# HITSZ-NRSL/De6D

Hardware: AMD Instinct MI355X
Metric: scenes/sec (16384-pt KITTI) at 1/2/4/8 MI355X; 3D mAP parity vs ref (higher is better)
Workload: dtype f32

## Files before the change

de6d_amd/csrc/mlp_chain.hip:

```cpp
#include "common.h"
#include <stdlib.h>

namespace {

D6_GEMM_PRIO_DECL

typedef float f32x16 __attribute__((ext_vector_type(16)));

constexpr int kChainWaves = 4;
constexpr int kPackTiles = 1;
constexpr int kTS = 33;
constexpr int kMaxK1 = 8;
constexpr int kMaxC = 32;
constexpr int kMaxC3 = 64;

struct ChainArgs {
  int rows;
  int n, m, ns;
  const float *a; int lda;
  const int *idx;
  const float *ctr; int ldctr;
  const int *cnt;
  const float *w1, *w2, *w3;
  int ldw1, ldw2, ldw3;
  const float *s1, *s2, *s3;
  int k1, c1, c2, c3;
  float *y; int ldy; int col0;
  const int *hdr; const int *crow_p; const int *crow_c;
};

__device__ __forceinline__ int compact_class(int row0, int h1, int h2, int h3, int h4, int h5) {
  return row0 < h1 ? 32 : row0 < h2 ? 16 : row0 < h3 ? 8 : row0 < h4 ? 4 : row0 < h5 ? 2 : 1;
}
__device__ __forceinline__ int compact_out_row(int s, int qq, int kh) {
  if (s < 4) return -1;
  if (s == 4) return 8 * qq + 4 * kh;
  if (kh) return -1;
  if (s == 8) return 8 * qq;
  if (s == 16) return (qq & 1) ? -1 : 8 * qq;
  return qq == 0 ? 0 : -1;
}
__device__ __forceinline__ void compact_store(float *dst, float val, int tag) {
  if (tag & 0x20000000) __hip_atomic_fetch_max(reinterpret_cast<int *>(dst), __builtin_bit_cast(int, val), __ATOMIC_RELAXED, __HIP_MEMORY_SCOPE_AGENT);
  else *dst = val;
}
__device__ __forceinline__ void compact_store_small(const ChainArgs &g, const f32x16 &o, int s, const int (&tags)[16], int col, float sh) {
#pragma unroll
  for (int e = 0; e < 16; ++e) {
    if (s == 2 && (e & 1)) continue;
    const float raw = s == 2 ? d6_vmax(o[e], o[e + 1 < 16 ? e + 1 : e]) : o[e];
    const int tag = tags[e];
    if (tag >= 0) compact_store(g.y + (size_t)(tag & 0x1fffffff) * g.ldy + g.col0 + col, (tag & 0x40000000) ? 0.f : d6_relu(raw + sh), tag);
  }
}
__device__ __forceinline__ void compact_row_tags(int my_tag, int kh, int (&tags)[16]) {
#pragma unroll
  for (int e = 0; e < 16; ++e) tags[e] = __shfl(my_tag, (e & 3) + 8 * (e >> 2) + 4 * kh);
}
__device__ __forceinline__ void compact_pool(float (&v)[4], int s) {
  if (s == 4) return;
#pragma unroll
  for (int qq = 0; qq < 4; ++qq) v[qq] = d6_vmax(v[qq], __shfl_xor(v[qq], 32));
  if (s == 16) {
    v[0] = d6_vmax(v[0], v[1]);
    v[2] = d6_vmax(v[2], v[3]);
  } else if (s == 32) {
    v[0] = d6_vmax(d6_vmax(v[0], v[1]), d6_vmax(v[2], v[3]));
  }
}

__device__ __forceinline__ float relu1(float v) { return v > 0.f ? v : 0.f; }

__host__ __device__ __forceinline__ int chain_col(int j, int k1) { return j + 3 < k1 ? j + 3 : j + 3 - k1; }

__global__ __launch_bounds__(64 * kChainWaves) void mlp_chain_kernel(const ChainArgs g) {
  D6_GEMM_PRIO_APPLY();
  __shared__ float W1[kMaxK1 * kMaxC];
  __shared__ float W2[kMaxC * kMaxC];
  __shared__ float W3[kMaxC * kMaxC3];
  __shared__ float S1[kMaxC], S2[kMaxC], S3[kMaxC3];
  __shared__ float T[kChainWaves][2][kMaxC * kTS];

  const int tid = threadIdx.x, lane = tid & 63, wave = tid >> 6;
  const int l31 = lane & 31, kh = lane >> 5;

  for (int t = tid; t < kMaxK1 * kMaxC; t += blockDim.x) {
    const int k = t / kMaxC, c = t % kMaxC;
    W1[t] = (k < g.k1 && c < g.c1) ? g.w1[(size_t)chain_col(k, g.k1) * g.ldw1 + c] : 0.f;
  }
  for (int t = tid; t < kMaxC * kMaxC; t += blockDim.x) {
    const int k = t / kMaxC, c = t % kMaxC;
// ... 94 lines not shown
      if (j >= nt3) break;
      const int col = 32 * j + l31;
      const bool cok = col < g.c3;
      const float sh = S3[col];
      float q[4];
#pragma unroll
      for (int qq = 0; qq < 4; ++qq) {
        float mx = relu1(acc3[j][4 * qq] + sh);
#pragma unroll
        for (int e = 1; e < 4; ++e) {
          const float v = relu1(acc3[j][4 * qq + e] + sh);
          mx = v > mx ? v : mx;
        }
        const float o = __shfl_xor(mx, 32);
        q[qq] = o > mx ? o : mx;
      }
      if (g.ns == 32) {
        float mx = q[0];
        mx = q[1] > mx ? q[1] : mx; mx = q[2] > mx ? q[2] : mx; mx = q[3] > mx ? q[3] : mx;
        if (cok && kh == 0) g.y[(size_t)tile * g.ldy + g.col0 + col] = (g.cnt[tile] > 0) ? mx : 0.f;
      } else {
        const float m0 = q[1] > q[0] ? q[1] : q[0];
        const float m1 = q[3] > q[2] ? q[3] : q[2];
        if (cok && kh == 0) {
          g.y[(size_t)(2 * tile) * g.ldy + g.col0 + col] = (g.cnt[2 * tile] > 0) ? m0 : 0.f;
          g.y[(size_t)(2 * tile + 1) * g.ldy + g.col0 + col] = (g.cnt[2 * tile + 1] > 0) ? m1 : 0.f;
        }
      }
    }
    __builtin_amdgcn_wave_barrier();
  }
}

template <int C1, int C2, int C3, int NS, bool COMPACT = false>
__global__ __launch_bounds__(256) void mlp_chain_reg_kernel(const ChainArgs g) {
  D6_GEMM_PRIO_APPLY();
  constexpr int S1 = 2;
  constexpr int S2 = C1 / 2, S3 = C2 / 2, NT3 = C3 / 32;
  const int lane = threadIdx.x & 63, l31 = lane & 31, kh = lane >> 5;
  int wave_global = (blockIdx.x * blockDim.x + threadIdx.x) >> 6;
  int n_waves = (gridDim.x * blockDim.x) >> 6;
  int pk_end = 0;
  if (COMPACT) {
    const int wpw = blockDim.x >> 6, live = g.hdr[0] / 32;
    int nb = (live + wpw * kPackTiles - 1) / (wpw * kPackTiles);
    if (nb > (int)gridDim.x) nb = gridDim.x;
    if ((int)blockIdx.x >= nb) return;
    n_waves = nb * wpw;
    pk_end = live;
  }

  float wf1[S1 + 1], wf2[S2 + 1], wf3[NT3][S3];
#pragma unroll
  for (int s = 0; s < S1; ++s) wf1[s] = l31 < C1 ? g.w1[(size_t)chain_col(2 * s + kh, 4) * g.ldw1 + l31] : 0.f;
  wf1[S1] = (kh == 0 && l31 < C1) ? g.s1[l31] : 0.f;
#pragma unroll
  for (int s = 0; s < S2; ++s) wf2[s] = l31 < C2 ? g.w2[(size_t)(2 * s + kh) * g.ldw2 + l31] : 0.f;
  wf2[S2] = (kh == 0 && l31 < C2) ? g.s2[l31] : 0.f;
#pragma unroll
  for (int j = 0; j < NT3; ++j)
#pragma unroll
    for (int s = 0; s < S3; ++s) wf3[j][s] = g.w3[(size_t)(2 * s + kh) * g.ldw3 + 32 * j + l31];
  float sh3[NT3];
#pragma unroll
  for (int j = 0; j < NT3; ++j) sh3[j] = g.s3[32 * j + l31];
  const float one_k0 = kh == 0 ? 1.f : 0.f;

  int h1 = 0, h2 = 0, h3 = 0, h4 = 0, h5 = 0;
  if (COMPACT) { h1 = g.hdr[1]; h2 = g.hdr[2]; h3 = g.hdr[3]; h4 = g.hdr[4]; h5 = g.hdr[5]; }
  const int ntiles = COMPACT ? pk_end : g.rows / 32;
  const int *nb_idx = COMPACT ? g.crow_p : g.idx;
  int tile = __builtin_amdgcn_readfirstlane(wave_global);
  if (tile >= ntiles) return;
  struct TileIn { float4 row; float cx, cy, cz; int cnt0, cnt1; int oc[4]; int tag; };
  struct TileIdx { int p, cj; };
  auto fetch_idx = [&](int t) {
    TileIdx ix;
    ix.p = nb_idx[t * 32 + l31];
    ix.cj = COMPACT ? g.crow_c[t * 32 + l31] : 0;
    return ix;
  };
  auto fetch = [&](int t, const TileIdx &ix) {
    TileIn in;
    const int p = ix.p;
    if (COMPACT) {
      in.row = *reinterpret_cast<const float4 *>(g.a + (size_t)p * 4);
      const int cj = ix.cj;
      const float *c = g.ctr + (size_t)(cj < 0 ? 0 : cj & 0x1fffffff) * g.ldctr;
      in.cx = c[0]; in.cy = c[1]; in.cz = c[2];
      in.cnt0 = in.cnt1 = 0;
      in.tag = cj;
      const int sc = compact_class(t * 32, h1, h2, h3, h4, h5);
#pragma unroll
      for (int qq = 0; qq < 4; ++qq) {
        const int r = compact_out_row(sc, qq, kh);
        const int tg = __shfl(cj, r < 0 ? 0 : r);
        in.oc[qq] = r >= 0 ? tg : -1;
      }
      return in;
    }
    in.tag = 0;
    const int c0 = NS == 32 ? t : 2 * t;
    const int bi = c0 / g.m;
    const int cj = NS == 32 ? c0 : c0 + (l31 >> 4);
    in.row = *reinterpret_cast<const float4 *>(g.a + ((size_t)bi * g.n + p) * 4);
    const float *c = g.ctr + (size_t)cj * g.ldctr;
    in.cx = c[0]; in.cy = c[1]; in.cz = c[2];
    in.cnt0 = g.cnt[c0];
    in.cnt1 = NS == 32 ? 0 : g.cnt[c0 + 1];
    return in;
  };
  TileIn nxt = fetch(tile, fetch_idx(tile));
  TileIdx ix_next = tile + n_waves < ntiles ? fetch_idx(tile + n_waves) : TileIdx{0, 0};
  float pend[NT3][COMPACT ? 4 : 2];
  int pend_oc[4] = {-1, -1, -1, -1};
  int pend_tile = -1;
  auto flush = [&]() {
#pragma unroll
    for (int j = 0; j < NT3; ++j) {
      const int col = 32 * j + l31;
      if (COMPACT) {
#pragma unroll
        for (int qq = 0; qq < 4; ++qq)
          if (pend_oc[qq] >= 0) compact_store(g.y + (size_t)(pend_oc[qq] & 0x1fffffff) * g.ldy + g.col0 + col, pend[j][qq], pend_oc[qq]);
      } else if (NS == 32) {
        g.y[(size_t)pend_tile * g.ldy + g.col0 + col] = pend[j][0];
      } else {
        g.y[(size_t)(2 * pend_tile) * g.ldy + g.col0 + col] = pend[j][0];
        g.y[(size_t)(2 * pend_tile + 1) * g.ldy + g.col0 + col] = pend[j][1];
      }
    }
  };
  for (; tile < ntiles; tile += n_waves) {
    const TileIn cur = nxt;
    if (pend_tile >= 0) flush();
    if (tile + n_waves < ntiles) {
      nxt = fetch(tile + n_waves, ix_next);
      if (tile + 2 * n_waves < ntiles) ix_next = fetch_idx(tile + 2 * n_waves);
    }
    const float4 v0 = cur.row;
    const float cx = cur.cx, cy = cur.cy, cz = cur.cz;
    const float x0 = v0.x - cx, x1 = v0.y - cy, x2 = v0.z - cz, x3 = v0.w;

    f32x16 acc;
#pragma unroll
    for (int e = 0; e < 16; ++e) acc[e] = 0.f;
    acc = __builtin_amdgcn_mfma_f32_32x32x2f32(wf1[0], kh ? x0 : x3, acc, 0, 0, 0);
    acc = __builtin_amdgcn_mfma_f32_32x32x2f32(wf1[1], kh ? x2 : x1, acc, 0, 0, 0);
    acc = __builtin_amdgcn_mfma_f32_32x32x2f32(wf1[2], one_k0, acc, 0, 0, 0);
    float frag[16];
    auto to_fragments = [&](const f32x16 &a, int nreg) {
#pragma unroll
      for (int G = 0; G < 4; ++G) {
        if (4 * G >= nreg) break;
        float t[4];
#pragma unroll
        for (int e = 0; e < 4; ++e) t[e] = d6_relu(a[4 * G + e]);
        asm volatile("s_nop 1\n\tv_permlane32_swap_b32 %0, %1\n\ts_nop 1\n\tv_permlane32_swap_b32 %2, %3\n\ts_nop 1"
                     : "+v"(t[0]), "+v"(t[1]), "+v"(t[2]), "+v"(t[3]));
        frag[4 * G + 0] = t[0];
        frag[4 * G + 1] = t[2];
        frag[4 * G + 2] = t[1];
        frag[4 * G + 3] = t[3];
      }
    };
    to_fragments(acc, S2);
#pragma unroll
    for (int e = 0; e < 16; ++e) acc[e] = 0.f;
#pragma unroll
    for (int s = 0; s < S2; ++s) acc = __builtin_amdgcn_mfma_f32_32x32x2f32(wf2[s], frag[s], acc, 0, 0, 0);
    acc = __builtin_amdgcn_mfma_f32_32x32x2f32(wf2[S2], one_k0, acc, 0, 0, 0);
    to_fragments(acc, S3);
#pragma unroll
    for (int j = 0; j < NT3; ++j) {
      f32x16 o;
#pragma unroll
      for (int e = 0; e < 16; ++e) o[e] = 0.f;
#pragma unroll
      for (int s = 0; s < S3; ++s) o = __builtin_amdgcn_mfma_f32_32x32x2f32(frag[s], wf3[j][s], o, 0, 0, 0);
      const int col = 32 * j + l31;
      float q[4];
      if (COMPACT) {
#pragma unroll
        for (int qq = 0; qq < 4; ++qq) q[qq] = d6_vmax(d6_vmax(o[4 * qq], o[4 * qq + 1]), d6_vmax(o[4 * qq + 2], o[4 * qq + 3]));
        const int sc = compact_class(tile * 32, h1, h2, h3, h4, h5);
        if (sc < 4) {
          int tags[16];
          compact_row_tags(cur.tag, kh, tags);
          compact_store_small(g, o, sc, tags, col, sh3[j]);
#pragma unroll
          for (int qq = 0; qq < 4; ++qq) pend[j][qq] = 0.f;
          continue;
        }
        compact_pool(q, sc);
#pragma unroll
        for (int qq = 0; qq < 4; ++qq) pend[j][qq] = (cur.oc[qq] & 0x40000000) ? 0.f : d6_relu(q[qq] + sh3[j]);
        continue;
      }
#pragma unroll
      for (int qq = 0; qq < 4; ++qq) {
        const float mq = d6_vmax(d6_vmax(o[4 * qq], o[4 * qq + 1]), d6_vmax(o[4 * qq + 2], o[4 * qq + 3]));
        q[qq] = d6_vmax(mq, __shfl_xor(mq, 32));
      }
      if (NS == 32) {
        const float mx = d6_relu(d6_vmax(d6_vmax(q[0], q[1]), d6_vmax(q[2], q[3])) + sh3[j]);
        pend[j][0] = (cur.cnt0 > 0) ? mx : 0.f;
      } else {
        const float m0 = d6_relu(d6_vmax(q[0], q[1]) + sh3[j]);
        const float m1 = d6_relu(d6_vmax(q[2], q[3]) + sh3[j]);
        pend[j][0] = (cur.cnt0 > 0) ? m0 : 0.f;
        pend[j][1] = (cur.cnt1 > 0) ? m1 : 0.f;
      }
    }
    pend_tile = tile;
    if (COMPACT) {
#pragma unroll
      for (int qq = 0; qq < 4; ++qq) pend_oc[qq] = cur.oc[qq];
    }
  }
  flush();
}

template <int N, int STRIDE, bool W_IS_A>
__device__ __forceinline__ void mfma_steps_lds(const float *__restrict__ w, const float *x, f32x16 &acc) {
  constexpr int UB = 8, NB = (N + UB - 1) / UB;
  float wb[2][UB];
#pragma unroll
  for (int u = 0; u < UB; ++u)
    if (u < N) wb[0][u] = w[u * STRIDE];
#pragma unroll
  for (int b = 0; b < NB; ++b) {
    if (b + 1 < NB) {
#pragma unroll
      for (int u = 0; u < UB; ++u)
        if ((b + 1) * UB + u < N) wb[(b + 1) & 1][u] = w[((b + 1) * UB + u) * STRIDE];
    }
    __builtin_amdgcn_sched_barrier(0);
#pragma unroll
    for (int u = 0; u < UB; ++u) {
      if (b * UB + u < N) {
        if (W_IS_A) acc = __builtin_amdgcn_mfma_f32_32x32x2f32(wb[b & 1][u], x[b * UB + u], acc, 0, 0, 0);
        else acc = __builtin_amdgcn_mfma_f32_32x32x2f32(x[b * UB + u], wb[b & 1][u], acc, 0, 0, 0);
      }
    }
    __builtin_amdgcn_sched_barrier(0);
  }
}

template <int C2, int NS, bool COMPACT = false>
__global__ __launch_bounds__(512) void mlp_chain_wide_kernel(const ChainArgs g) {
  D6_GEMM_PRIO_APPLY();
  constexpr int K1 = 68, C1 = 64, C3 = 128;
  constexpr int S1 = K1 / 2, S2 = C1 / 2, S3 = C2 / 2;
  constexpr int T1 = C1 / 32, T2 = C2 / 32, T3 = C3 / 32;
  extern __shared__ float lds[];
  float *W1 = lds;
  float *W2 = W1 + (K1 + 2) * C1;
  float *W3 = W2 + (C1 + 2) * C2;
  const int tid = threadIdx.x, lane = tid & 63, l31 = lane & 31, kh = lane >> 5;
  int pk_stride = 0, pk_first = 0, pk_end = 0;
  if (COMPACT) {
    const int wpw = blockDim.x >> 6, live = g.hdr[0] / 32;
    int nb = (live + wpw * kPackTiles - 1) / (wpw * kPackTiles);
    if (nb > (int)gridDim.x) nb = gridDim.x;
    if ((int)blockIdx.x >= nb) return;
    pk_stride = nb * wpw;
    pk_first = blockIdx.x * wpw + (tid >> 6);
    pk_end = live;
  }
  auto stage = [&](float *dst, const float *w, int ldw, const float *shift, int k_rows, int cols, bool chain_order) {
    const int c4 = cols / 4;
    for (int t = tid; t < (k_rows + (shift ? 2 : 0)) * c4; t += blockDim.x) {
      const int k = t / c4, c = 4 * (t % c4);
      float4 v = make_float4(0.f, 0.f, 0.f, 0.f);
      if (k < k_rows) v = *reinterpret_cast<const float4 *>(w + (size_t)(chain_order ? chain_col(k, k_rows) : k) * ldw + c);
      else if (k == k_rows) v = *reinterpret_cast<const float4 *>(shift + c);
      *reinterpret_cast<float4 *>(dst + k * cols + c) = v;
    }
  };
  stage(W1, g.w1, g.ldw1, g.s1, K1, C1, true);
  stage(W2, g.w2, g.ldw2, g.s2, C1, C2, false);
  stage(W3, g.w3, g.ldw3, nullptr, C2, C3, false);
  float sh3[T3];
#pragma unroll
  for (int j = 0; j < T3; ++j) sh3[j] = g.s3[32 * j + l31];
  __syncthreads();

  const float one_k0 = kh == 0 ? 1.f : 0.f;
  const int wave_global = COMPACT ? pk_first : (int)((blockIdx.x * blockDim.x + tid) >> 6);
  const int n_waves = COMPACT ? pk_stride : (int)((gridDim.x * blockDim.x) >> 6);
  int h1 = 0, h2 = 0, h3 = 0, h4 = 0, h5 = 0;
  if (COMPACT) { h1 = g.hdr[1]; h2 = g.hdr[2]; h3 = g.hdr[3]; h4 = g.hdr[4]; h5 = g.hdr[5]; }
  const int ntiles = COMPACT ? pk_end : g.rows / 32;
  int tile = __builtin_amdgcn_readfirstlane(wave_global);
  if (tile >= ntiles) return;

  float xin[S1 + 1];
  float csub0, csub1;
  int cnt0, cnt1;
  int oc_n[4] = {-1, -1, -1, -1};
  int e_p = 0, e_c = 0, tag_n = 0;
  auto fetch_entries = [&](int t) {
    if (COMPACT) {
      e_p = g.crow_p[t * 32 + l31];
      e_c = g.crow_c[t * 32 + l31];
    } else {
      e_p = g.idx[t * 32 + l31];
    }
  };
  auto fetch = [&](int t) {
    if (COMPACT) {
      const int p = e_p;
      const float *row = g.a + (size_t)p * K1;
      const float *src = row + 3 + kh;
#pragma unroll
      for (int s = 0; s < S1 - 2; ++s) xin[s] = src[2 * s];
      xin[S1 - 2] = row[kh ? 0 : K1 - 1];
      xin[S1 - 1] = row[kh ? 2 : 1];
      const int cj = e_c;
      const float *c = g.ctr + (size_t)(cj < 0 ? 0 : cj & 0x1fffffff) * g.ldctr;
      csub0 = kh ? c[0] : 0.f;
      csub1 = kh ? c[2] : c[1];
      cnt0 = cnt1 = 0;
      tag_n = cj;
      const int sc = compact_class(t * 32, h1, h2, h3, h4, h5);
#pragma unroll
      for (int qq = 0; qq < 4; ++qq) {
        const int r = compact_out_row(sc, qq, kh);
        const int tg = __shfl(cj, r < 0 ? 0 : r);
        oc_n[qq] = r >= 0 ? tg : -1;
      }
      return;
    }
    const int c0 = NS == 32 ? t : 2 * t;
    const int bi = c0 / g.m;
    const int cj = NS == 32 ? c0 : c0 + (l31 >> 4);
    const int p = e_p;
    const float *row = g.a + ((size_t)bi * g.n + p) * K1;
    const float *src = row + 3 + kh;
#pragma unroll
    for (int s = 0; s < S1 - 2; ++s) xin[s] = src[2 * s];
    xin[S1 - 2] = row[kh ? 0 : K1 - 1];
    xin[S1 - 1] = row[kh ? 2 : 1];
    const float *c = g.ctr + (size_t)cj * g.ldctr;
    csub0 = kh ? c[0] : 0.f;
    csub1 = kh ? c[2] : c[1];
    cnt0 = g.cnt[c0];
    cnt1 = NS == 32 ? 0 : g.cnt[c0 + 1];
  };
  auto to_fragments = [&](const f32x16 &a, float *frag) {
#pragma unroll
    for (int G = 0; G < 4; ++G) {
      float t[4];
#pragma unroll
      for (int e = 0; e < 4; ++e) t[e] = d6_relu(a[4 * G + e]);
      asm volatile("s_nop 1\n\tv_permlane32_swap_b32 %0, %1\n\ts_nop 1\n\tv_permlane32_swap_b32 %2, %3\n\ts_nop 1"
                   : "+v"(t[0]), "+v"(t[1]), "+v"(t[2]), "+v"(t[3]));
      frag[4 * G + 0] = t[0]; frag[4 * G + 1] = t[2]; frag[4 * G + 2] = t[1]; frag[4 * G + 3] = t[3];
    }
  };

  float pend[T3][COMPACT ? 4 : 2];
  int pend_oc[4] = {-1, -1, -1, -1};
  int pend_tile = -1;
  auto flush = [&]() {
#pragma unroll
    for (int j = 0; j < T3; ++j) {
      const int col = 32 * j + l31;
      if (COMPACT) {
#pragma unroll
        for (int qq = 0; qq < 4; ++qq)
          if (pend_oc[qq] >= 0) compact_store(g.y + (size_t)(pend_oc[qq] & 0x1fffffff) * g.ldy + g.col0 + col, pend[j][qq], pend_oc[qq]);
      } else if (NS == 32) {
        g.y[(size_t)pend_tile * g.ldy + g.col0 + col] = pend[j][0];
      } else {
        g.y[(size_t)(2 * pend_tile) * g.ldy + g.col0 + col] = pend[j][0];
        g.y[(size_t)(2 * pend_tile + 1) * g.ldy + g.col0 + col] = pend[j][1];
      }
    }
  };

  fetch_entries(tile);
  fetch(tile);
  if (tile + n_waves < ntiles) fetch_entries(tile + n_waves);
  for (; tile < ntiles; tile += n_waves) {
    if (pend_tile >= 0) flush();
    const int my_cnt0 = cnt0, my_cnt1 = cnt1, my_tag = tag_n;
    int my_oc[4];
#pragma unroll
    for (int qq = 0; qq < 4; ++qq) my_oc[qq] = oc_n[qq];
    xin[S1 - 2] = xin[S1 - 2] - csub0;
    xin[S1 - 1] = xin[S1 - 1] - csub1;
    xin[S1] = one_k0;
    float f1[S2 + 1];
#pragma unroll
    for (int t = 0; t < T1; ++t) {
      f32x16 acc;
#pragma unroll
      for (int e = 0; e < 16; ++e) acc[e] = 0.f;
      mfma_steps_lds<S1 + 1, 2 * C1, true>(W1 + kh * C1 + 32 * t + l31, xin, acc);
      to_fragments(acc, f1 + 16 * t);
    }
    f1[S2] = one_k0;
    if (tile + n_waves < ntiles) {
      fetch(tile + n_waves);
      if (tile + 2 * n_waves < ntiles) fetch_entries(tile + 2 * n_waves);
    }
    float f2[S3];
#pragma unroll
    for (int t = 0; t < T2; ++t) {
      f32x16 acc;
#pragma unroll
      for (int e = 0; e < 16; ++e) acc[e] = 0.f;
      mfma_steps_lds<S2 + 1, 2 * C2, true>(W2 + kh * C2 + 32 * t + l31, f1, acc);
      to_fragments(acc, f2 + 16 * t);
    }
#pragma unroll
    for (int j = 0; j < T3; ++j) {
      f32x16 o;
#pragma unroll
      for (int e = 0; e < 16; ++e) o[e] = 0.f;
      mfma_steps_lds<S3, 2 * C3, false>(W3 + kh * C3 + 32 * j + l31, f2, o);
      float q[4];
      if (COMPACT) {
#pragma unroll
        for (int qq = 0; qq < 4; ++qq) q[qq] = d6_vmax(d6_vmax(o[4 * qq], o[4 * qq + 1]), d6_vmax(o[4 * qq + 2], o[4 * qq + 3]));
        const int sc = compact_class(tile * 32, h1, h2, h3, h4, h5);
        if (sc < 4) {
          int tags[16];
          compact_row_tags(my_tag, kh, tags);
          compact_store_small(g, o, sc, tags, 32 * j + l31, sh3[j]);
#pragma unroll
          for (int qq = 0; qq < 4; ++qq) pend[j][qq] = 0.f;
          continue;
        }
        compact_pool(q, sc);
#pragma unroll
        for (int qq = 0; qq < 4; ++qq) pend[j][qq] = (my_oc[qq] & 0x40000000) ? 0.f : d6_relu(q[qq] + sh3[j]);
        continue;
      }
#pragma unroll
      for (int qq = 0; qq < 4; ++qq) {
        const float mq = d6_vmax(d6_vmax(o[4 * qq], o[4 * qq + 1]), d6_vmax(o[4 * qq + 2], o[4 * qq + 3]));
        q[qq] = d6_vmax(mq, __shfl_xor(mq, 32));
      }
      if (NS == 32) {
        const float mx = d6_relu(d6_vmax(d6_vmax(q[0], q[1]), d6_vmax(q[2], q[3])) + sh3[j]);
        pend[j][0] = my_cnt0 > 0 ? mx : 0.f;
      } else {
        pend[j][0] = my_cnt0 > 0 ? d6_relu(d6_vmax(q[0], q[1]) + sh3[j]) : 0.f;
        pend[j][1] = my_cnt1 > 0 ? d6_relu(d6_vmax(q[2], q[3]) + sh3[j]) : 0.f;
      }
    }
    pend_tile = tile;
    if (COMPACT) {
#pragma unroll
      for (int qq = 0; qq < 4; ++qq) pend_oc[qq] = my_oc[qq];
    }
  }
  flush();
}

}

DET6D_API int det6d_mlp_chain3(int rows, int n, int m, int ns, const float *a, int lda, const int *idx,
                               const float *ctr, int ldctr, const int *cnt, const float *w1, int ldw1,
                               const float *s1, int c1, const float *w2, int ldw2, const float *s2, int c2,
                               const float *w3, int ldw3, const float *s3, int c3, float *y, int ldy, int col0,
                               det6d_stream_t stream) {
  D6_GEMM_PRIO_HOST();
  if (rows < 0 || n <= 0 || m <= 0 || (ns != 16 && ns != 32) || !a || !idx || !ctr || !cnt || !w1 || !w2 || !w3 ||
      !s1 || !s2 || !s3 || !y)
    return DET6D_EINVAL;
  const bool wide = lda == 68 && c1 == 64 && (c2 == 64 || c2 == 96) && c3 == 128 && (ns == 32 || !(m & 1)) && !(ldw1 & 3) &&
                    !(ldw2 & 3) && !(ldw3 & 3) &&
                    !(((uintptr_t)w1 | (uintptr_t)w2 | (uintptr_t)w3 | (uintptr_t)s1 | (uintptr_t)s2) & 15) &&
                    !det6d_env_set("DET6D_CHAIN_NO_WIDE");
  if (!wide) {
    if (lda < 4 || lda > kMaxK1 || (lda & 3) || ((uintptr_t)a & 15) || ldctr < 3) return DET6D_EINVAL;
    if (c1 <= 0 || c1 > kMaxC || c2 <= 0 || c2 > kMaxC || c3 <= 0 || c3 > kMaxC3) return DET6D_EINVAL;
  }
  if (ldw1 < c1 || ldw2 < c2 || ldw3 < c3 || rows % (m * ns) || rows % 32) return DET6D_EINVAL;
  if (rows == 0) return DET6D_OK;
  ChainArgs g;
  g.rows = rows; g.n = n; g.m = m; g.ns = ns;
  g.a = a; g.lda = lda; g.idx = idx; g.ctr = ctr; g.ldctr = ldctr; g.cnt = cnt;
  g.w1 = w1; g.w2 = w2; g.w3 = w3; g.ldw1 = ldw1; g.ldw2 = ldw2; g.ldw3 = ldw3;
  g.s1 = s1; g.s2 = s2; g.s3 = s3;
  g.k1 = lda; g.c1 = c1; g.c2 = c2; g.c3 = c3;
  g.y = y; g.ldy = ldy; g.col0 = col0;
  g.hdr = nullptr; g.crow_p = nullptr; g.crow_c = nullptr;
  const int ntiles = rows / 32;
  if (wide) {
    const size_t lds_bytes = sizeof(float) * ((size_t)70 * 64 + (size_t)66 * c2 + (size_t)c2 * 128);
    const int wb = det6d_divup(ntiles, 8) < 256 ? det6d_divup(ntiles, 8) : 256;
#define D6_WIDE(C2V, NSV)                                                                                              \
  do {                                                                                                                 \
    DET6D_MAX_DYNAMIC_LDS((mlp_chain_wide_kernel<C2V, NSV>), lds_bytes);                                               \
    hipLaunchKernelGGL((mlp_chain_wide_kernel<C2V, NSV>), dim3(wb), dim3(512), lds_bytes, (hipStream_t)stream, g);     \
  } while (0)
    if (c2 == 64 && ns == 16) D6_WIDE(64, 16);
    else if (c2 == 64) D6_WIDE(64, 32);
    else if (ns == 16) D6_WIDE(96, 16);
    else D6_WIDE(96, 32);
#undef D6_WIDE
    return det6d_check_launch("det6d_mlp_chain3");
  }
  int blocks = det6d_divup(ntiles, kChainWaves);
  if (blocks > 256 * 6) blocks = 256 * 6;
  static const bool use_lds_env = det6d_env_set("DET6D_CHAIN_LDS");
  const bool use_lds = use_lds_env || (ns == 16 && (m & 1));
  static const int reg_blocks_env = det6d_env_int("DET6D_CHAIN_BLOCKS", 1024);
  const int reg_blocks = blocks < reg_blocks_env ? blocks : reg_blocks_env;
  if (!use_lds && lda == 4 && c1 == 16 && c2 == 16 && c3 == 32 && ns == 16)
    hipLaunchKernelGGL((mlp_chain_reg_kernel<16, 16, 32, 16>), dim3(reg_blocks), dim3(256), 0, (hipStream_t)stream, g);
  else if (!use_lds && lda == 4 && c1 == 16 && c2 == 16 && c3 == 32 && ns == 32)
    hipLaunchKernelGGL((mlp_chain_reg_kernel<16, 16, 32, 32>), dim3(reg_blocks), dim3(256), 0, (hipStream_t)stream, g);
  else if (!use_lds && lda == 4 && c1 == 32 && c2 == 32 && c3 == 64 && ns == 16)
    hipLaunchKernelGGL((mlp_chain_reg_kernel<32, 32, 64, 16>), dim3(reg_blocks), dim3(256), 0, (hipStream_t)stream, g);
  else if (!use_lds && lda == 4 && c1 == 32 && c2 == 32 && c3 == 64 && ns == 32)
    hipLaunchKernelGGL((mlp_chain_reg_kernel<32, 32, 64, 32>), dim3(reg_blocks), dim3(256), 0, (hipStream_t)stream, g);
  else
    hipLaunchKernelGGL(mlp_chain_kernel, dim3(blocks), dim3(64 * kChainWaves), 0, (hipStream_t)stream, g);
  return det6d_check_launch("det6d_mlp_chain3");
}

DET6D_API int det6d_mlp_chain3_compact(int capacity, const int *hdr, const int *crow_p, const int *crow_c, const float *a,
                                       int lda, const float *ctr, int ldctr, const float *w1, int ldw1, const float *s1,
                                       int c1, const float *w2, int ldw2, const float *s2, int c2, const float *w3, int ldw3,
                                       const float *s3, int c3, float *y, int ldy, int col0, det6d_stream_t stream) {
  D6_GEMM_PRIO_HOST();
  if (capacity <= 0 || (capacity & 127) || !hdr || !crow_p || !crow_c || !a || !ctr || ldctr < 3 || !w1 || !w2 || !w3 || !s1 ||
      !s2 || !s3 || !y)
    return DET6D_EINVAL;
  if (ldw1 < c1 || ldw2 < c2 || ldw3 < c3) return DET6D_EINVAL;
  const bool wide = lda == 68 && c1 == 64 && (c2 == 64 || c2 == 96) && c3 == 128 && !(ldw1 & 3) && !(ldw2 & 3) && !(ldw3 & 3) &&
                    !(((uintptr_t)w1 | (uintptr_t)w2 | (uintptr_t)w3 | (uintptr_t)s1 | (uintptr_t)s2) & 15);
  const bool narrow = lda == 4 && !((uintptr_t)a & 15) && ((c1 == 16 && c2 == 16 && c3 == 32) || (c1 == 32 && c2 == 32 && c3 == 64));
  if (!wide && !narrow) return DET6D_EINVAL;
  ChainArgs g;
  g.rows = capacity; g.n = 0; g.m = 0; g.ns = 0;
  g.a = a; g.lda = lda; g.idx = nullptr; g.ctr = ctr; g.ldctr = ldctr; g.cnt = nullptr;
  g.w1 = w1; g.w2 = w2; g.w3 = w3; g.ldw1 = ldw1; g.ldw2 = ldw2; g.ldw3 = ldw3;
  g.s1 = s1; g.s2 = s2; g.s3 = s3;
  g.k1 = lda; g.c1 = c1; g.c2 = c2; g.c3 = c3;
  g.y = y; g.ldy = ldy; g.col0 = col0;
  g.hdr = hdr; g.crow_p = crow_p; g.crow_c = crow_c;
  const int ntiles = capacity / 32;
  if (wide) {
    const size_t lds_bytes = sizeof(float) * ((size_t)70 * 64 + (size_t)66 * c2 + (size_t)c2 * 128);
    const int wb = det6d_divup(ntiles, 8) < 256 ? det6d_divup(ntiles, 8) : 256;
    if (c2 == 64) {
      DET6D_MAX_DYNAMIC_LDS((mlp_chain_wide_kernel<64, 32, true>), lds_bytes);
      hipLaunchKernelGGL((mlp_chain_wide_kernel<64, 32, true>), dim3(wb), dim3(512), lds_bytes, (hipStream_t)stream, g);
    } else {
      DET6D_MAX_DYNAMIC_LDS((mlp_chain_wide_kernel<96, 32, true>), lds_bytes);
      hipLaunchKernelGGL((mlp_chain_wide_kernel<96, 32, true>), dim3(wb), dim3(512), lds_bytes, (hipStream_t)stream, g);
    }
    return det6d_check_launch("det6d_mlp_chain3_compact");
  }
  int blocks = det6d_divup(ntiles, 4);
  static const int cap = det6d_env_int("DET6D_CHAIN_BLOCKS", 2048);
  if (blocks > cap) blocks = cap;
  if (c1 == 16)
    hipLaunchKernelGGL((mlp_chain_reg_kernel<16, 16, 32, 32, true>), dim3(blocks), dim3(256), 0, (hipStream_t)stream, g);
  else
    hipLaunchKernelGGL((mlp_chain_reg_kernel<32, 32, 64, 32, true>), dim3(blocks), dim3(256), 0, (hipStream_t)stream, g);
  return det6d_check_launch("det6d_mlp_chain3_compact");
}
```

Before: 12850.

## Use buffer stores with wave-uniform masks for compact MLP chain scatter

Reworks the compact-path output scatter in the MLP chain kernels. Row tags are no longer shuffled per element. They are turned into wave-level ballot masks and per-row byte offsets, and outputs go through raw buffer stores and buffer atomic smax with 32-bit offsets. In the wide and paired-register kernels it also swaps two 32-column halves with v_permlane32_swap so each lane writes whole rows, and it adds a fallback 64-bit-address kernel instantiation for outputs that exceed 4 GiB. The aim is to cut shuffle and address arithmetic, and to get more coalesced stores. The cost is more complex code, inline asm and a second launch when the buffer is large.

```diff
diff --git a/de6d_amd/csrc/mlp_chain.hip b/de6d_amd/csrc/mlp_chain.hip
--- a/de6d_amd/csrc/mlp_chain.hip
+++ b/de6d_amd/csrc/mlp_chain.hip
@@ -1,5 +1,8 @@
 #include "common.h"
 #include <stdlib.h>
+
+__device__ int det6d_chain_buffer_atomic_smax(int v, __amdgpu_buffer_rsrc_t rsrc, int voffset, int soffset, int aux)
+    __asm("llvm.amdgcn.raw.ptr.buffer.atomic.smax.i32");
 
 namespace {
 
@@ -27,7 +30,10 @@
   int k1, c1, c2, c3;
   float *y; int ldy; int col0;
   const int *hdr; const int *crow_p; const int *crow_c;
+  int pick32;
 };
+
+__host__ __device__ __forceinline__ bool compact_fits32(long long centres, int ldy) { return centres * ldy * 4ll <= 0xffffffffll; }
 
 __device__ __forceinline__ int compact_class(int row0, int h1, int h2, int h3, int h4, int h5) {
   return row0 < h1 ? 32 : row0 < h2 ? 16 : row0 < h3 ? 8 : row0 < h4 ? 4 : row0 < h5 ? 2 : 1;
@@ -40,23 +46,183 @@
   if (s == 16) return (qq & 1) ? -1 : 8 * qq;
   return qq == 0 ? 0 : -1;
 }
-__device__ __forceinline__ void compact_store(float *dst, float val, int tag) {
-  if (tag & 0x20000000) __hip_atomic_fetch_max(reinterpret_cast<int *>(dst), __builtin_bit_cast(int, val), __ATOMIC_RELAXED, __HIP_MEMORY_SCOPE_AGENT);
-  else *dst = val;
-}
-__device__ __forceinline__ void compact_store_small(const ChainArgs &g, const f32x16 &o, int s, const int (&tags)[16], int col, float sh) {
+struct CompactTile {
+  uint32_t plain;
+  uint32_t store;
+  uint32_t atomic;
+  uint32_t empty;
+  uint32_t off;
+};
+
+__device__ __forceinline__ int chain_acc_row(int e, int kh) { return (e & 3) + 8 * (e >> 2) + 4 * kh; }
+__device__ __forceinline__ bool chain_halves(uint32_t lo, uint32_t hi) {
+  return __builtin_amdgcn_inverse_ballot_w64((unsigned long long)lo | (unsigned long long)hi << 32);
+}
+__device__ __forceinline__ uint32_t chain_bit(uint32_t m, int r) { return r < 0 ? 0u : 0u - (m >> r & 1u); }
+__device__ __forceinline__ uint32_t chain_fresh(uint32_t x, int j) { return __builtin_amdgcn_readfirstlane(x ^ (uint32_t)(j + 1)) ^ (uint32_t)(j + 1); }
+
+__device__ __forceinline__ CompactTile compact_tile(int tag, uint32_t row_mul) {
+  CompactTile ct;
+  const bool live = tag >= 0;
+  const uint32_t pad = (uint32_t)__ballot(!live), split = (uint32_t)__ballot(live && (tag & 0x20000000));
+  ct.empty = (uint32_t)__ballot(live && (tag & 0x40000000));
+  ct.store = ~pad & ~split;
+  ct.atomic = ~pad & split;
+  ct.plain = ct.store & ~ct.empty;
+  ct.off = live ? (uint32_t)(tag & 0x1fffffff) * row_mul : 0u;
+  return ct;
+}
+__device__ __forceinline__ void compact_atomic(float *dst, float val) {
+  __hip_atomic_fetch_max(reinterpret_cast<int *>(dst), __builtin_bit_cast(int, val), __ATOMIC_RELAXED, __HIP_MEMORY_SCOPE_AGENT);
+}
+template <bool FITS32>
+__device__ __forceinline__ void compact_put(const ChainArgs &g, const __amdgpu_buffer_rsrc_t srd, bool whole, uint32_t st_lo, uint32_t st_hi,
+                                            uint32_t at_lo, uint32_t at_hi, uint32_t zero_lo, uint32_t zero_hi, float val, uint32_t off,
+                                            int col) {
+  if constexpr (FITS32) {
+    if (whole) {
+      __builtin_amdgcn_raw_buffer_store_b32(__float_as_uint(val), srd, off, 0, 0);
+    } else {
+      const float v = chain_halves(zero_lo, zero_hi) ? 0.f : val;
+      if (chain_halves(st_lo, st_hi)) __builtin_amdgcn_raw_buffer_store_b32(__float_as_uint(v), srd, off, 0, 0);
+      if (chain_halves(at_lo, at_hi)) det6d_chain_buffer_atomic_smax(__builtin_bit_cast(int, v), srd, off, 0, 0);
+    }
+  } else {
+    float *dst = g.y + (size_t)off * g.ldy + g.col0 + col;
+    const float v = chain_halves(zero_lo, zero_hi) ? 0.f : val;
+    if (whole || chain_halves(st_lo, st_hi)) *dst = v;
+    if (!whole && chain_halves(at_lo, at_hi)) compact_atomic(dst, v);
+  }
+}
+template <bool FITS32>
+__device__ __forceinline__ void compact_store_small(const ChainArgs &g, const __amdgpu_buffer_rsrc_t srd, const CompactTile &ct, int s, int j,
+                                                    const f32x16 &o, int kh, int l31, float sh) {
+  const uint32_t lane_colb = FITS32 ? (uint32_t)(g.col0 + l31) * 4u : 0u;
+  const int col = 32 * j + l31;
+  const uint32_t plain = chain_fresh(ct.plain, j), store = chain_fresh(ct.store, j), atomic = chain_fresh(ct.atomic, j),
+                 empty = chain_fresh(ct.empty, j);
+  const int src0 = s < 3 ? 16 * kh : 0;
+  const int row_off = (int)(ct.off + (FITS32 ? 128u * j : 0u));
 #pragma unroll
   for (int e = 0; e < 16; ++e) {
     if (s == 2 && (e & 1)) continue;
     const float raw = s == 2 ? d6_vmax(o[e], o[e + 1 < 16 ? e + 1 : e]) : o[e];
-    const int tag = tags[e];
-    if (tag >= 0) compact_store(g.y + (size_t)(tag & 0x1fffffff) * g.ldy + g.col0 + col, (tag & 0x40000000) ? 0.f : d6_relu(raw + sh), tag);
-  }
-}
-__device__ __forceinline__ void compact_row_tags(int my_tag, int kh, int (&tags)[16]) {
-#pragma unroll
-  for (int e = 0; e < 16; ++e) tags[e] = __shfl(my_tag, (e & 3) + 8 * (e >> 2) + 4 * kh);
-}
+    const int ra = chain_acc_row(e, 0), rb = chain_acc_row(e, 1);
+    const uint32_t m = 1u << ra | 1u << rb;
+    const uint32_t off = (uint32_t)__builtin_amdgcn_ds_bpermute(src0 + 4 * ra, row_off) + lane_colb;
+    compact_put<FITS32>(g, srd, (plain & m) == m, chain_bit(store, ra), chain_bit(store, rb), chain_bit(atomic, ra), chain_bit(atomic, rb),
+                        chain_bit(empty, ra), chain_bit(empty, rb), d6_relu(raw + sh), off, col);
+  }
+}
+struct CompactPend { uint32_t row_off; uint32_t bits; bool both; };
+
+__device__ __forceinline__ CompactPend compact_pend(const CompactTile &ct, int s) {
+  CompactPend p;
+  p.row_off = ct.off;
+  p.bits = 0u;
+  p.both = s == 4;
+#pragma unroll
+  for (int qq = 0; qq < 4; ++qq) {
+    const int ra = compact_out_row(s, qq, 0), rb = compact_out_row(s, qq, 1);
+    p.bits |= ((chain_bit(ct.store, ra) & 1u) | (chain_bit(ct.store, rb) & 2u) | (chain_bit(ct.atomic, ra) & 4u) | (chain_bit(ct.atomic, rb) & 8u))
+              << (4 * qq);
+  }
+  return p;
+}
+__device__ __forceinline__ bool compact_pend_empty(const CompactTile &ct, int s, int qq) {
+  return chain_halves(chain_bit(ct.empty, compact_out_row(s, qq, 0)), chain_bit(ct.empty, compact_out_row(s, qq, 1)));
+}
+template <bool FITS32, int NT>
+__device__ __forceinline__ void compact_flush(const ChainArgs &g, const __amdgpu_buffer_rsrc_t srd, const CompactPend &p, const float (&vals)[NT][4],
+                                              int col0, int l31, int kh) {
+  if (p.bits == 0u) return;
+  const int src0 = p.both ? 16 * kh : 0;
+  const uint32_t lane_colb = FITS32 ? (uint32_t)(col0 + l31) * 4u : 0u;
+#pragma unroll
+  for (int qq = 0; qq < 4; ++qq) {
+    const uint32_t b = p.bits >> (4 * qq);
+    const uint32_t off = (uint32_t)__builtin_amdgcn_ds_bpermute(src0 + 32 * qq, (int)p.row_off) + lane_colb;
+#pragma unroll
+    for (int j = 0; j < NT; ++j)
+      compact_put<FITS32>(g, srd, (b & 3u) == 3u, chain_bit(b, 0), chain_bit(b, 1), chain_bit(b, 2), chain_bit(b, 3), 0u, 0u, vals[j][qq],
+                          off + (FITS32 ? 128u * j : 0u), 32 * j + l31);
+  }
+}
+
+__device__ __forceinline__ int compact_row_mode(uint32_t store, uint32_t atomic, uint32_t empty, int r) {
+  if (r < 0) return 0;
+  return (store >> r & 1u) ? ((empty >> r & 1u) ? 3 : 1) : (atomic >> r & 1u) ? 2 : 0;
+}
+__device__ __forceinline__ void chain_swap_halves(float &a, float &b) {
+  asm volatile("s_nop 1\n\tv_permlane32_swap_b32 %0, %1\n\ts_nop 1" : "+v"(a), "+v"(b));
+}
+template <bool FITS32>
+__device__ __forceinline__ void compact_put_row(const ChainArgs &g, const __amdgpu_buffer_rsrc_t srd, int mode, float val, uint32_t voff,
+                                                uint32_t row, int col) {
+  if (mode == 0) return;
+  const float v = mode == 3 ? 0.f : val;
+  if constexpr (FITS32) {
+    if (mode == 2) det6d_chain_buffer_atomic_smax(__builtin_bit_cast(int, v), srd, voff, row, 0);
+    else __builtin_amdgcn_raw_buffer_store_b32(__float_as_uint(v), srd, voff, row, 0);
+  } else {
+    float *dst = g.y + (size_t)row * g.ldy + g.col0 + col;
+    if (mode == 2) compact_atomic(dst, v);
+    else *dst = v;
+  }
+}
+template <bool FITS32>
+__device__ __forceinline__ void compact_store_small_pair(const ChainArgs &g, const __amdgpu_buffer_rsrc_t srd, const CompactTile &ct, int s, int j,
+                                                         const f32x16 &oa, const f32x16 &ob, int lane, float sha, float shb) {
+  const uint32_t store = chain_fresh(ct.store, j), atomic = chain_fresh(ct.atomic, j), empty = chain_fresh(ct.empty, j);
+  const int col = 32 * j + lane;
+  const uint32_t voff = (uint32_t)(g.col0 + col) * 4u;
+  const float sh = lane < 32 ? sha : shb;
+#pragma unroll
+  for (int e = 0; e < 16; ++e) {
+    if (s == 2 && (e & 1)) continue;
+    float a = s == 2 ? d6_vmax(oa[e], oa[e + 1 < 16 ? e + 1 : e]) : oa[e];
+    float b = s == 2 ? d6_vmax(ob[e], ob[e + 1 < 16 ? e + 1 : e]) : ob[e];
+    chain_swap_halves(a, b);
+    const int ra = chain_acc_row(e, 0), rb = chain_acc_row(e, 1);
+    compact_put_row<FITS32>(g, srd, compact_row_mode(store, atomic, empty, ra), d6_relu(a + sh), voff, __builtin_amdgcn_readlane(ct.off, ra), col);
+    compact_put_row<FITS32>(g, srd, compact_row_mode(store, atomic, empty, rb), d6_relu(b + sh), voff, __builtin_amdgcn_readlane(ct.off, rb), col);
+  }
+}
+struct CompactPendRows { uint32_t row_off; uint32_t modes; int s; };
+
+__device__ __forceinline__ CompactPendRows compact_pend_rows(const CompactTile &ct, int s) {
+  CompactPendRows p;
+  p.row_off = ct.off;
+  p.s = s;
+  p.modes = 0u;
+#pragma unroll
+  for (int qq = 0; qq < 4; ++qq)
+    p.modes |= (uint32_t)(compact_row_mode(ct.store, ct.atomic, ct.empty, compact_out_row(s, qq, 0)) |
+                          compact_row_mode(ct.store, ct.atomic, ct.empty, compact_out_row(s, qq, 1)) << 2)
+               << (4 * qq);
+  return p;
+}
+template <bool FITS32, int NT>
+__device__ __forceinline__ void compact_flush_rows(const ChainArgs &g, const __amdgpu_buffer_rsrc_t srd, const CompactPendRows &p,
+                                                   const float (&vals)[NT][4], int lane) {
+  if (p.modes == 0u) return;
+#pragma unroll
+  for (int qq = 0; qq < 4; ++qq) {
+    const int ra = compact_out_row(p.s, qq, 0), rb = compact_out_row(p.s, qq, 1);
+    const int ma = p.modes >> (4 * qq) & 3, mb = p.modes >> (4 * qq + 2) & 3;
+    const uint32_t row_a = __builtin_amdgcn_readlane(p.row_off, ra < 0 ? 0 : ra), row_b = __builtin_amdgcn_readlane(p.row_off, rb < 0 ? 0 : rb);
+#pragma unroll
+    for (int j = 0; j < NT; j += 2) {
+      float a = vals[j][qq], b = vals[j + 1][qq];
+      chain_swap_halves(a, b);
+      const int col = 32 * j + lane;
+      const uint32_t voff = (uint32_t)(g.col0 + col) * 4u;
+      compact_put_row<FITS32>(g, srd, ma, a, voff, row_a, col);
+      compact_put_row<FITS32>(g, srd, mb, b, voff, row_b, col);
+    }
+  }
+}
+
 __device__ __forceinline__ void compact_pool(float (&v)[4], int s) {
   if (s == 4) return;
 #pragma unroll
@@ -217,7 +383,7 @@
   }
 }
 
-template <int C1, int C2, int C3, int NS, bool COMPACT = false>
+template <int C1, int C2, int C3, int NS, bool COMPACT = false, bool FITS32 = true>
 __global__ __launch_bounds__(256) void mlp_chain_reg_kernel(const ChainArgs g) {
   D6_GEMM_PRIO_APPLY();
   constexpr int S1 = 2;
@@ -227,6 +393,7 @@
   int n_waves = (gridDim.x * blockDim.x) >> 6;
   int pk_end = 0;
   if (COMPACT) {
+    if (g.pick32 && compact_fits32(g.hdr[7], g.ldy) != FITS32) return;
     const int wpw = blockDim.x >> 6, live = g.hdr[0] / 32;
     int nb = (live + wpw * kPackTiles - 1) / (wpw * kPackTiles);
     if (nb > (int)gridDim.x) nb = gridDim.x;
@@ -257,7 +424,7 @@
   const int *nb_idx = COMPACT ? g.crow_p : g.idx;
   int tile = __builtin_amdgcn_readfirstlane(wave_global);
   if (tile >= ntiles) return;
-  struct TileIn { float4 row; float cx, cy, cz; int cnt0, cnt1; int oc[4]; int tag; };
+  struct TileIn { float4 row; float cx, cy, cz; int cnt0, cnt1; int tag; };
   struct TileIdx { int p, cj; };
   auto fetch_idx = [&](int t) {
     TileIdx ix;
@@ -275,13 +442,6 @@
       in.cx = c[0]; in.cy = c[1]; in.cz = c[2];
       in.cnt0 = in.cnt1 = 0;
       in.tag = cj;
-      const int sc = compact_class(t * 32, h1, h2, h3, h4, h5);
-#pragma unroll
-      for (int qq = 0; qq < 4; ++qq) {
-        const int r = compact_out_row(sc, qq, kh);
-        const int tg = __shfl(cj, r < 0 ? 0 : r);
-        in.oc[qq] = r >= 0 ? tg : -1;
-      }
       return in;
     }
     in.tag = 0;
@@ -298,17 +458,26 @@
   TileIn nxt = fetch(tile, fetch_idx(tile));
   TileIdx ix_next = tile + n_waves < ntiles ? fetch_idx(tile + n_waves) : TileIdx{0, 0};
   float pend[NT3][COMPACT ? 4 : 2];
-  int pend_oc[4] = {-1, -1, -1, -1};
+  constexpr bool PAIRS = COMPACT && NT3 % 2 == 0;
+  CompactPend pend_c;
+  pend_c.bits = 0u; pend_c.both = false; pend_c.row_off = 0u;
+  CompactPendRows pend_r;
+  pend_r.modes = 0u; pend_r.s = 4; pend_r.row_off = 0u;
   int pend_tile = -1;
+  const __amdgpu_buffer_rsrc_t srd_y = __builtin_amdgcn_make_buffer_rsrc((void *)g.y, 0, 0xffffffff, 0x00020000);
+  const uint32_t row_mul = FITS32 ? (uint32_t)g.ldy * 4u : 1u;
   auto flush = [&]() {
+    if constexpr (PAIRS) {
+      compact_flush_rows<FITS32, NT3>(g, srd_y, pend_r, pend, lane);
+      return;
+    } else if constexpr (COMPACT) {
+      compact_flush<FITS32, NT3>(g, srd_y, pend_c, pend, g.col0, l31, kh);
+      return;
+    }
 #pragma unroll
     for (int j = 0; j < NT3; ++j) {
       const int col = 32 * j + l31;
-      if (COMPACT) {
-#pragma unroll
-        for (int qq = 0; qq < 4; ++qq)
-          if (pend_oc[qq] >= 0) compact_store(g.y + (size_t)(pend_oc[qq] & 0x1fffffff) * g.ldy + g.col0 + col, pend[j][qq], pend_oc[qq]);
-      } else if (NS == 32) {
+      if (NS == 32) {
         g.y[(size_t)pend_tile * g.ldy + g.col0 + col] = pend[j][0];
       } else {
         g.y[(size_t)(2 * pend_tile) * g.ldy + g.col0 + col] = pend[j][0];
@@ -356,8 +525,50 @@
     for (int s = 0; s < S2; ++s) acc = __builtin_amdgcn_mfma_f32_32x32x2f32(wf2[s], frag[s], acc, 0, 0, 0);
     acc = __builtin_amdgcn_mfma_f32_32x32x2f32(wf2[S2], one_k0, acc, 0, 0, 0);
     to_fragments(acc, S3);
-#pragma unroll
-    for (int j = 0; j < NT3; ++j) {
+    const int sc = COMPACT ? compact_class(tile * 32, h1, h2, h3, h4, h5) : 0;
+    CompactTile ct;
+    if (COMPACT) {
+      ct = compact_tile(cur.tag, row_mul);
+      if (sc < 4) {
+        pend_c.bits = 0u;
+        pend_r.modes = 0u;
+      } else if (PAIRS) {
+        pend_r = compact_pend_rows(ct, sc);
+      } else {
+        pend_c = compact_pend(ct, sc);
+      }
+    }
+    if constexpr (PAIRS) {
+#pragma unroll
+      for (int j = 0; j < NT3; j += 2) {
+        f32x16 oa, ob;
+#pragma unroll
+        for (int e = 0; e < 16; ++e) oa[e] = ob[e] = 0.f;
+#pragma unroll
+        for (int s = 0; s < S3; ++s) oa = __builtin_amdgcn_mfma_f32_32x32x2f32(frag[s], wf3[j][s], oa, 0, 0, 0);
+#pragma unroll
+        for (int s = 0; s < S3; ++s) ob = __builtin_amdgcn_mfma_f32_32x32x2f32(frag[s], wf3[j + 1][s], ob, 0, 0, 0);
+        if (sc < 4) {
+          compact_store_small_pair<FITS32>(g, srd_y, ct, sc, j, oa, ob, lane, sh3[j], sh3[j + 1]);
+          continue;
+        }
+        float qa[4], qb[4];
+#pragma unroll
+        for (int qq = 0; qq < 4; ++qq) {
+          qa[qq] = d6_vmax(d6_vmax(oa[4 * qq], oa[4 * qq + 1]), d6_vmax(oa[4 * qq + 2], oa[4 * qq + 3]));
+          qb[qq] = d6_vmax(d6_vmax(ob[4 * qq], ob[4 * qq + 1]), d6_vmax(ob[4 * qq + 2], ob[4 * qq + 3]));
+        }
+        compact_pool(qa, sc);
+        compact_pool(qb, sc);
+#pragma unroll
+        for (int qq = 0; qq < 4; ++qq) {
+          pend[j][qq] = d6_relu(qa[qq] + sh3[j]);
+          pend[j + 1][qq] = d6_relu(qb[qq] + sh3[j + 1]);
+        }
+      }
+    }
+#pragma unroll
+    for (int j = 0; j < (PAIRS ? 0 : NT3); ++j) {
       f32x16 o;
 #pragma unroll
       for (int e = 0; e < 16; ++e) o[e] = 0.f;
@@ -368,18 +579,13 @@
       if (COMPACT) {
 #pragma unroll
         for (int qq = 0; qq < 4; ++qq) q[qq] = d6_vmax(d6_vmax(o[4 * qq], o[4 * qq + 1]), d6_vmax(o[4 * qq + 2], o[4 * qq + 3]));
-        const int sc = compact_class(tile * 32, h1, h2, h3, h4, h5);
         if (sc < 4) {
-          int tags[16];
-          compact_row_tags(cur.tag, kh, tags);
-          compact_store_small(g, o, sc, tags, col, sh3[j]);
-#pragma unroll
-          for (int qq = 0; qq < 4; ++qq) pend[j][qq] = 0.f;
+          compact_store_small<FITS32>(g, srd_y, ct, sc, j, o, kh, l31, sh3[j]);
           continue;
         }
         compact_pool(q, sc);
 #pragma unroll
-        for (int qq = 0; qq < 4; ++qq) pend[j][qq] = (cur.oc[qq] & 0x40000000) ? 0.f : d6_relu(q[qq] + sh3[j]);
+        for (int qq = 0; qq < 4; ++qq) pend[j][qq] = compact_pend_empty(ct, sc, qq) ? 0.f : d6_relu(q[qq] + sh3[j]);
         continue;
       }
 #pragma unroll
@@ -398,10 +604,6 @@
       }
     }
     pend_tile = tile;
-    if (COMPACT) {
-#pragma unroll
-      for (int qq = 0; qq < 4; ++qq) pend_oc[qq] = cur.oc[qq];
-    }
   }
   flush();
 }
@@ -432,7 +634,7 @@
   }
 }
 
-template <int C2, int NS, bool COMPACT = false>
+template <int C2, int NS, bool COMPACT = false, bool FITS32 = true>
 __global__ __launch_bounds__(512) void mlp_chain_wide_kernel(const ChainArgs g) {
   D6_GEMM_PRIO_APPLY();
   constexpr int K1 = 68, C1 = 64, C3 = 128;
@@ -445,6 +647,7 @@
   const int tid = threadIdx.x, lane = tid & 63, l31 = lane & 31, kh = lane >> 5;
   int pk_stride = 0, pk_first = 0, pk_end = 0;
   if (COMPACT) {
+    if (g.pick32 && compact_fits32(g.hdr[7], g.ldy) != FITS32) return;
     const int wpw = blockDim.x >> 6, live = g.hdr[0] / 32;
     int nb = (live + wpw * kPackTiles - 1) / (wpw * kPackTiles);
     if (nb > (int)gridDim.x) nb = gridDim.x;
@@ -483,7 +686,6 @@
   float xin[S1 + 1];
   float csub0, csub1;
   int cnt0, cnt1;
-  int oc_n[4] = {-1, -1, -1, -1};
   int e_p = 0, e_c = 0, tag_n = 0;
   auto fetch_entries = [&](int t) {
     if (COMPACT) {
@@ -508,13 +710,6 @@
       csub1 = kh ? c[2] : c[1];
       cnt0 = cnt1 = 0;
       tag_n = cj;
-      const int sc = compact_class(t * 32, h1, h2, h3, h4, h5);
-#pragma unroll
-      for (int qq = 0; qq < 4; ++qq) {
-        const int r = compact_out_row(sc, qq, kh);
-        const int tg = __shfl(cj, r < 0 ? 0 : r);
-        oc_n[qq] = r >= 0 ? tg : -1;
-      }
       return;
     }
     const int c0 = NS == 32 ? t : 2 * t;
@@ -546,17 +741,20 @@
   };
 
   float pend[T3][COMPACT ? 4 : 2];
-  int pend_oc[4] = {-1, -1, -1, -1};
+  CompactPendRows pend_r;
+  pend_r.modes = 0u; pend_r.s = 4; pend_r.row_off = 0u;
   int pend_tile = -1;
+  const __amdgpu_buffer_rsrc_t srd_y = __builtin_amdgcn_make_buffer_rsrc((void *)g.y, 0, 0xffffffff, 0x00020000);
+  const uint32_t row_mul = FITS32 ? (uint32_t)g.ldy * 4u : 1u;
   auto flush = [&]() {
+    if constexpr (COMPACT) {
+      compact_flush_rows<FITS32, T3>(g, srd_y, pend_r, pend, lane);
+      return;
+    }
 #pragma unroll
     for (int j = 0; j < T3; ++j) {
       const int col = 32 * j + l31;
-      if (COMPACT) {
-#pragma unroll
-        for (int qq = 0; qq < 4; ++qq)
-          if (pend_oc[qq] >= 0) compact_store(g.y + (size_t)(pend_oc[qq] & 0x1fffffff) * g.ldy + g.col0 + col, pend[j][qq], pend_oc[qq]);
-      } else if (NS == 32) {
+      if (NS == 32) {
         g.y[(size_t)pend_tile * g.ldy + g.col0 + col] = pend[j][0];
       } else {
         g.y[(size_t)(2 * pend_tile) * g.ldy + g.col0 + col] = pend[j][0];
@@ -570,10 +768,9 @@
   if (tile + n_waves < ntiles) fetch_entries(tile + n_waves);
   for (; tile < ntiles; tile += n_waves) {
     if (pend_tile >= 0) flush();
-    const int my_cnt0 = cnt0, my_cnt1 = cnt1, my_tag = tag_n;
-    int my_oc[4];
-#pragma unroll
-    for (int qq = 0; qq < 4; ++qq) my_oc[qq] = oc_n[qq];
+    const int my_cnt0 = cnt0, my_cnt1 = cnt1;
+    CompactTile ct;
+    if (COMPACT) ct = compact_tile(tag_n, row_mul);
     xin[S1 - 2] = xin[S1 - 2] - csub0;
     xin[S1 - 1] = xin[S1 - 1] - csub1;
     xin[S1] = one_k0;
@@ -600,30 +797,43 @@
       mfma_steps_lds<S2 + 1, 2 * C2, true>(W2 + kh * C2 + 32 * t + l31, f1, acc);
       to_fragments(acc, f2 + 16 * t);
     }
-#pragma unroll
-    for (int j = 0; j < T3; ++j) {
+    const int sc = COMPACT ? compact_class(tile * 32, h1, h2, h3, h4, h5) : 0;
+    if constexpr (COMPACT) {
+      if (sc < 4) pend_r.modes = 0u;
+      else pend_r = compact_pend_rows(ct, sc);
+#pragma unroll
+      for (int j = 0; j < T3; j += 2) {
+        f32x16 oa, ob;
+#pragma unroll
+        for (int e = 0; e < 16; ++e) oa[e] = ob[e] = 0.f;
+        mfma_steps_lds<S3, 2 * C3, false>(W3 + kh * C3 + 32 * j + l31, f2, oa);
+        mfma_steps_lds<S3, 2 * C3, false>(W3 + kh * C3 + 32 * (j + 1) + l31, f2, ob);
+        if (sc < 4) {
+          compact_store_small_pair<FITS32>(g, srd_y, ct, sc, j, oa, ob, lane, sh3[j], sh3[j + 1]);
+          continue;
+        }
+        float qa[4], qb[4];
+#pragma unroll
+        for (int qq = 0; qq < 4; ++qq) {
+          qa[qq] = d6_vmax(d6_vmax(oa[4 * qq], oa[4 * qq + 1]), d6_vmax(oa[4 * qq + 2], oa[4 * qq + 3]));
+          qb[qq] = d6_vmax(d6_vmax(ob[4 * qq], ob[4 * qq + 1]), d6_vmax(ob[4 * qq + 2], ob[4 * qq + 3]));
+        }
+        compact_pool(qa, sc);
+        compact_pool(qb, sc);
+#pragma unroll
+        for (int qq = 0; qq < 4; ++qq) {
+          pend[j][qq] = d6_relu(qa[qq] + sh3[j]);
+          pend[j + 1][qq] = d6_relu(qb[qq] + sh3[j + 1]);
+        }
+      }
+    }
+#pragma unroll
+    for (int j = 0; j < (COMPACT ? 0 : T3); ++j) {
       f32x16 o;
 #pragma unroll
       for (int e = 0; e < 16; ++e) o[e] = 0.f;
       mfma_steps_lds<S3, 2 * C3, false>(W3 + kh * C3 + 32 * j + l31, f2, o);
       float q[4];
-      if (COMPACT) {
-#pragma unroll
-        for (int qq = 0; qq < 4; ++qq) q[qq] = d6_vmax(d6_vmax(o[4 * qq], o[4 * qq + 1]), d6_vmax(o[4 * qq + 2], o[4 * qq + 3]));
-        const int sc = compact_class(tile * 32, h1, h2, h3, h4, h5);
-        if (sc < 4) {
-          int tags[16];
-          compact_row_tags(my_tag, kh, tags);
-          compact_store_small(g, o, sc, tags, 32 * j + l31, sh3[j]);
-#pragma unroll
-          for (int qq = 0; qq < 4; ++qq) pend[j][qq] = 0.f;
-          continue;
-        }
-        compact_pool(q, sc);
-#pragma unroll
-        for (int qq = 0; qq < 4; ++qq) pend[j][qq] = (my_oc[qq] & 0x40000000) ? 0.f : d6_relu(q[qq] + sh3[j]);
-        continue;
-      }
 #pragma unroll
       for (int qq = 0; qq < 4; ++qq) {
         const float mq = d6_vmax(d6_vmax(o[4 * qq], o[4 * qq + 1]), d6_vmax(o[4 * qq + 2], o[4 * qq + 3]));
@@ -638,10 +848,6 @@
       }
     }
     pend_tile = tile;
-    if (COMPACT) {
-#pragma unroll
-      for (int qq = 0; qq < 4; ++qq) pend_oc[qq] = my_oc[qq];
-    }
   }
   flush();
 }
@@ -674,7 +880,7 @@
   g.s1 = s1; g.s2 = s2; g.s3 = s3;
   g.k1 = lda; g.c1 = c1; g.c2 = c2; g.c3 = c3;
   g.y = y; g.ldy = ldy; g.col0 = col0;
-  g.hdr = nullptr; g.crow_p = nullptr; g.crow_c = nullptr;
+  g.hdr = nullptr; g.crow_p = nullptr; g.crow_c = nullptr; g.pick32 = 0;
   const int ntiles = rows / 32;
   if (wide) {
     const size_t lds_bytes = sizeof(float) * ((size_t)70 * 64 + (size_t)66 * c2 + (size_t)c2 * 128);
@@ -719,6 +925,7 @@
       !s2 || !s3 || !y)
     return DET6D_EINVAL;
   if (ldw1 < c1 || ldw2 < c2 || ldw3 < c3) return DET6D_EINVAL;
+  if (col0 < 0 || c3 <= 0 || (long long)col0 + c3 > ldy || !compact_fits32(1, ldy)) return DET6D_EINVAL;
   const bool wide = lda == 68 && c1 == 64 && (c2 == 64 || c2 == 96) && c3 == 128 && !(ldw1 & 3) && !(ldw2 & 3) && !(ldw3 & 3) &&
                     !(((uintptr_t)w1 | (uintptr_t)w2 | (uintptr_t)w3 | (uintptr_t)s1 | (uintptr_t)s2) & 15);
   const bool narrow = lda == 4 && !((uintptr_t)a & 15) && ((c1 == 16 && c2 == 16 && c3 == 32) || (c1 == 32 && c2 == 32 && c3 == 64));
@@ -731,25 +938,35 @@
   g.k1 = lda; g.c1 = c1; g.c2 = c2; g.c3 = c3;
   g.y = y; g.ldy = ldy; g.col0 = col0;
   g.hdr = hdr; g.crow_p = crow_p; g.crow_c = crow_c;
+  g.pick32 = compact_fits32(capacity, ldy) ? 0 : 1;
   const int ntiles = capacity / 32;
   if (wide) {
     const size_t lds_bytes = sizeof(float) * ((size_t)70 * 64 + (size_t)66 * c2 + (size_t)c2 * 128);
     const int wb = det6d_divup(ntiles, 8) < 256 ? det6d_divup(ntiles, 8) : 256;
+#define D6_WIDE_COMPACT(C2V, F32)                                                                                      \
+  do {                                                                                                                 \
+    DET6D_MAX_DYNAMIC_LDS((mlp_chain_wide_kernel<C2V, 32, true, F32>), lds_bytes);                                     \
+    hipLaunchKernelGGL((mlp_chain_wide_kernel<C2V, 32, true, F32>), dim3(wb), dim3(512), lds_bytes, (hipStream_t)stream, g); \
+  } while (0)
     if (c2 == 64) {
-      DET6D_MAX_DYNAMIC_LDS((mlp_chain_wide_kernel<64, 32, true>), lds_bytes);
-      hipLaunchKernelGGL((mlp_chain_wide_kernel<64, 32, true>), dim3(wb), dim3(512), lds_bytes, (hipStream_t)stream, g);
+      D6_WIDE_COMPACT(64, true);
+      if (g.pick32) D6_WIDE_COMPACT(64, false);
     } else {
-      DET6D_MAX_DYNAMIC_LDS((mlp_chain_wide_kernel<96, 32, true>), lds_bytes);
-      hipLaunchKernelGGL((mlp_chain_wide_kernel<96, 32, true>), dim3(wb), dim3(512), lds_bytes, (hipStream_t)stream, g);
-    }
+      D6_WIDE_COMPACT(96, true);
+      if (g.pick32) D6_WIDE_COMPACT(96, false);
+    }
+#undef D6_WIDE_COMPACT
     return det6d_check_launch("det6d_mlp_chain3_compact");
   }
   int blocks = det6d_divup(ntiles, 4);
   static const int cap = det6d_env_int("DET6D_CHAIN_BLOCKS", 2048);
   if (blocks > cap) blocks = cap;
-  if (c1 == 16)
-    hipLaunchKernelGGL((mlp_chain_reg_kernel<16, 16, 32, 32, true>), dim3(blocks), dim3(256), 0, (hipStream_t)stream, g);
-  else
-    hipLaunchKernelGGL((mlp_chain_reg_kernel<32, 32, 64, 32, true>), dim3(blocks), dim3(256), 0, (hipStream_t)stream, g);
+  if (c1 == 16) {
+    hipLaunchKernelGGL((mlp_chain_reg_kernel<16, 16, 32, 32, true, true>), dim3(blocks), dim3(256), 0, (hipStream_t)stream, g);
+    if (g.pick32) hipLaunchKernelGGL((mlp_chain_reg_kernel<16, 16, 32, 32, true, false>), dim3(blocks), dim3(256), 0, (hipStream_t)stream, g);
+  } else {
+    hipLaunchKernelGGL((mlp_chain_reg_kernel<32, 32, 64, 32, true, true>), dim3(blocks), dim3(256), 0, (hipStream_t)stream, g);
+    if (g.pick32) hipLaunchKernelGGL((mlp_chain_reg_kernel<32, 32, 64, 32, true, false>), dim3(blocks), dim3(256), 0, (hipStream_t)stream, g);
+  }
   return det6d_check_launch("det6d_mlp_chain3_compact");
 }
```

New measurement: 12860 (median of 3 runs). About the same (+0.1%).
